# broadinstitute/gatk-bwamem-jni

Measured on AMD Instinct MI355X. Metric: 150bp reads aligned/sec vs GRCh38-scale reference (1/2/4/8 MI355X), higher is better.
Workload: dtype u8/int32/int64; 1 GPU; 10000000 x 150bp single-end synthetic reads per GPU vs synthetic GRCh38-scale genome (3100000000 bp, 24 contigs, 5% diverged repeats), full index in HBM; reads_per_gpu=10000000, read_len=150, genome_bp=3100000000, genome=iid, response_bytes=542940344, parallelism=read-sharded x1, no collectives, hip_hw_queues=4, paired_end=False

## Files before the change

### gatk-bwamem-jni_amd/csrc/bwamem_types.h

```cpp
#pragma once
#include <stdint.h>
#include <stddef.h>
#include <hip/hip_runtime.h>

struct MemOpt {
    int a, b;
    int o_del, e_del;
    int o_ins, e_ins;
    int pen_unpaired;
    int pen_clip5, pen_clip3;
    int w;
    int zdrop;
    uint64_t max_mem_intv;
    int T;
    int flag;
    int min_seed_len;
    int min_chain_weight;
    int max_chain_extend;
    float split_factor;
    int split_width;
    int max_occ;
    int max_chain_gap;
    int n_threads;
    int chunk_size;
// ... 56 lines not shown
    int64_t rb, re;
    int32_t qb, qe;
    int32_t rid;
    int32_t score, truesc, sub, alt_sc, csub, sub_n, w, seedcov, secondary, secondary_all, seedlen0;
    int32_t n_comp, is_alt;
    float frac_rep;
    int32_t pad_;
    uint64_t hash;
};

struct SwJob { int64_t rb; int32_t read, tag, l_ms, is_rev, tlen, xtra, q_off, pad_; };
struct KswR { int score, te, qe, score2, te2, tb, qb; };

struct DevCounters {
    unsigned long long n_ext, n_lf, n_sa, n_dp_cells, n_ref_bases, n_reads;
    unsigned long long dbg[10];
};

enum { ERR_INTV_CAP = 1, ERR_OUT_CAP = 2, ERR_CIGAR_CAP = 4, ERR_LONG_READ = 8, ERR_SCRATCH = 16, ERR_BTREE = 32, ERR_BAD_REG = 64, ERR_JOB_CAP = 128, ERR_ZPOOL = 256, ERR_RESCUE_CAP = 512 };

#define BT_NODE_INTS 40

struct TileView {
    int32_t n_reads;
    int32_t max_len;
    int64_t read_id0;
    const int64_t* seq_off;
    uint8_t* seq;
    int32_t intv_cap;
    Intv* intv;
    int32_t* n_intv;
// ... 36 lines not shown
```

### gatk-bwamem-jni_amd/csrc/k_cigar.hip

```cpp
#include "dev_common.h"
#include "wave_ops.h"
#include "kernels.h"
#include "post_common.h"

#define NEG_SCAN (-2000000000)

struct GClk { unsigned long long* c; long long t; };
DEV void gclk(GClk& K, int k) { if (K.c) { const long long t = clock64(); if (threadIdx.x == 0) atomicAdd(K.c + k, (unsigned long long)(t - K.t)); K.t = clock64(); } }

struct GLds { int32_t* eh_h; int32_t* eh_e; int32_t* tmpM; int rm; };


static __device__ __forceinline__ int traceback(const uint8_t* z, bool z_lds, int n_col, int w, int tlen, int qlen, int lane, uint32_t* cigar, int cig_cap, int& err, uint8_t* tile, GClk& K)
{
    gclk(K, 5);
    int n = 0;
    int which = 0, i = tlen - 1, k = (i + w + 1 < qlen ? i + w + 1 : qlen) - 1;
    int cur_op = -1;
    uint32_t cur_len = 0;
    bool ovf = false;
#define TB_PUSH(OP, LEN) do { if ((OP) == cur_op) cur_len += (uint32_t)(LEN); else { \
        if (cur_len) { if (n >= cig_cap) ovf = true; else { if (lane == 0) cigar[n] = cur_len << 4 | (uint32_t)cur_op; ++n; } } cur_op = (OP); cur_len = (uint32_t)(LEN); } } while (0)
#define TB_WALK(AVAIL, GET) \
    while (i >= 0 && k >= 0 && !ovf && AVAIL(i, k)) { \
// ... 256 lines not shown
    return score;
}

struct GRowTab { uint32_t p[5]; int n[5]; };
DEV GRowTab g_row_tab(const MemOpt& opt)
{
    GRowTab T;
#pragma unroll
    for (int t = 0; t < 5; ++t) {
        T.p[t] = (uint32_t)(uint8_t)opt.mat[t * 5] | (uint32_t)(uint8_t)opt.mat[t * 5 + 1] << 8 | (uint32_t)(uint8_t)opt.mat[t * 5 + 2] << 16 | (uint32_t)(uint8_t)opt.mat[t * 5 + 3] << 24;
        T.n[t] = opt.mat[t * 5 + 4];
    }
    return T;
}

template <int WMAX>
__global__ void __launch_bounds__(64, 2) k_gcigar_lane(DevIndex ix, MemOpt opt, TileView tv, const DpJob* jobs, DpOut* outs, int n_jobs, uint32_t* cig_pool, int cig_cap,
                                                    uint8_t* zpool, unsigned long long zpool_cap, unsigned long long* zpool_cur)
{
    constexpr int NS = 2 * WMAX + 1;
    constexpr int ZW = (NS + 7) / 8;
    const int job = blockIdx.x * 64 + threadIdx.x;
    if (job >= n_jobs) return;
    const DpJob jb = jobs[job];
    const AlnReg ar = tv.regs[tv.seed_off[jb.read] + jb.reg];
    const uint8_t* query = tv.seq + tv.seq_off[jb.read];
    SeqAcc A; A.q = query + ar.qb; A.qlen = ar.qe - ar.qb; A.rev = ar.rb >= ix.l_pac; A.t0 = ar.rb; A.tlen = (int)(ar.re - ar.rb);
    const int qlen = A.qlen, tlen = A.tlen;
    DpOut o; o.score = 0; o.n_cigar = -1;
    const bool usable = !(qlen <= 0 || ar.rb >= ar.re || (ar.rb < ix.l_pac && ar.re > ix.l_pac) || ar.re > ix.l_pac << 1 || ar.rb < 0);
    int w2 = first_w2(opt, ar), w = 0;
    if (usable) {
        w2 = w2 < opt.w << 2 ? w2 : opt.w << 2;
        int max_ins = div_plus(((qlen + 1) >> 1) * opt.mat[0] - opt.o_ins, opt.e_ins, 1);
        int max_del = div_plus(((qlen + 1) >> 1) * opt.mat[0] - opt.o_del, opt.e_del, 1);
        int max_gap = max_ins > max_del ? max_ins : max_del;
        max_gap = max_gap > 1 ? max_gap : 1;
        int d = tlen - qlen; d = d < 0 ? -d : d;
        w = (max_gap + d + 1) >> 1;
        w = w < w2 ? w : w2;
        const int min_w = d + 3;
        w = w > min_w ? w : min_w;
    }
    const int l_end = qlen - 1 - (tlen - 1 - w);
    uint32_t* z = 0;
    bool take = usable && w <= WMAX && l_end >= 0 && l_end <= 2 * w;
    if (take) {
        const unsigned long long need = ((unsigned long long)tlen * ZW * 4 + 63ull) & ~63ull;
        const unsigned long long at = atomicAdd(zpool_cur, need);
        if (at + need > zpool_cap) { atomicOr(tv.err, ERR_ZPOOL); take = false; }
        else z = (uint32_t*)(zpool + at);
    }
    if (!take) { outs[job] = o; return; }

    const int o_del = opt.o_del, e_del = opt.e_del, o_ins = opt.o_ins, e_ins = opt.e_ins;
    const int oe_del = o_del + e_del, oe_ins = o_ins + e_ins;
    const GRowTab RT = g_row_tab(opt);
    SeqCache sc; seq_cache_init(sc);
    int H[NS], E[NS], Q[NS];
#pragma unroll
    for (int l = 0; l < NS; ++l) {
        const int j0 = l - w;
        H[l] = j0 == 0 ? 0 : (j0 > 0 && j0 <= w ? -(o_ins + e_ins * j0) : MINUS_INF);
        E[l] = MINUS_INF;
        Q[l] = j0 >= 0 && j0 < qlen ? acc_q_c(A, sc, j0) : 4;
    }
    for (int i = 0; i < tlen; ++i) {
        const int tb = acc_t_c(ix, A, sc, i);
        const uint32_t R = tb == 0 ? RT.p[0] : tb == 1 ? RT.p[1] : tb == 2 ? RT.p[2] : tb == 3 ? RT.p[3] : RT.p[4];
        const int Rn = tb == 0 ? RT.n[0] : tb == 1 ? RT.n[1] : tb == 2 ? RT.n[2] : tb == 3 ? RT.n[3] : RT.n[4];
        const int c0 = i - w;
        const int hb = -(o_del + e_del * (i + 1));
        int f = MINUS_INF;
        uint32_t zw[ZW];
#pragma unroll
        for (int k = 0; k < ZW; ++k) zw[k] = 0;
#pragma unroll
        for (int l = 0; l < NS; ++l) {
            const int j = c0 + l;
            const bool act = j >= 0 && j < qlen && l <= 2 * w;
            const int q = Q[l];
            const int s = q < 4 ? (int)(int8_t)(R >> (q << 3)) : Rn;
            const int m = H[l] + s, e = E[l];
            int d = m >= e ? 0 : 1;
            int h = m >= e ? m : e;
            d = h >= f ? d : 2;
            h = h >= f ? h : f;
            const int t = m - oe_del;
            int e2 = e - e_del;
            d |= e2 > t ? 4 : 0;
            e2 = e2 > t ? e2 : t;
            const int t2 = m - oe_ins;
            int f2 = f - e_ins;
            d |= f2 > t2 ? 8 : 0;
            f2 = f2 > t2 ? f2 : t2;
            H[l] = act ? h : (j == -1 ? hb : MINUS_INF);
            if (l > 0) E[l - 1] = act ? e2 : MINUS_INF;
            f = act ? f2 : f;
            zw[l >> 3] |= act ? (uint32_t)d << ((l & 7) << 2) : 0u;
        }
        E[NS - 1] = MINUS_INF;
#pragma unroll
        for (int k = 0; k < ZW; ++k) z[i * ZW + k] = zw[k];
        const int inj = i + 1 - w + NS - 1;
        const int qin = inj >= 0 && inj < qlen ? acc_q_c(A, sc, inj) : 4;
#pragma unroll
        for (int l = 0; l + 1 < NS; ++l) Q[l] = Q[l + 1];
        Q[NS - 1] = qin;
    }
    int score = MINUS_INF;
#pragma unroll
    for (int l = 0; l < NS; ++l) score = l == l_end ? H[l] : score;

    if (!(w2 == opt.w << 2) && score < ar.truesc - opt.a) { outs[job] = o; return; }

    uint32_t* cigar = cig_pool + (size_t)job * cig_cap;
    int n = 0, cur_op = -1, which = 0, i = tlen - 1, k = (i + w + 1 < qlen ? i + w + 1 : qlen) - 1;
    uint32_t cur_len = 0;
    bool ovf = false;
#define TB_PUSH(OP, LEN) do { if ((OP) == cur_op) cur_len += (uint32_t)(LEN); else { \
        if (cur_len) { if (n >= cig_cap) ovf = true; else cigar[n++] = cur_len << 4 | (uint32_t)cur_op; } cur_op = (OP); cur_len = (uint32_t)(LEN); } } while (0)
    while (i >= 0 && k >= 0 && !ovf) {
        const int l = k - (i - w);
        const uint32_t nib = z[i * ZW + (l >> 3)] >> ((l & 7) << 2) & 15u;
        which = which == 0 ? (int)(nib & 3u) : which == 1 ? (int)(nib >> 2 & 1u) : (int)(nib >> 3 & 1u) << 1;
        if (which == 0) { TB_PUSH(0, 1); --i; --k; }
        else if (which == 1) { TB_PUSH(2, 1); --i; }
        else { TB_PUSH(1, 1); --k; }
    }
    if (!ovf && i >= 0) TB_PUSH(2, i + 1);
    if (!ovf && k >= 0) TB_PUSH(1, k + 1);
    if (!ovf) TB_PUSH(-1, 0);
#undef TB_PUSH
    for (int a = 0; a < n >> 1; ++a) { uint32_t tmp = cigar[a]; cigar[a] = cigar[n - 1 - a]; cigar[n - 1 - a] = tmp; }
    if (ovf) { atomicOr(tv.err, ERR_CIGAR_CAP); n = 0; }
    o.score = score; o.n_cigar = n;
    outs[job] = o;
}

template <bool HBM, int MAXCH>
__global__ void __launch_bounds__(64, MAXCH >= 13 ? 2 : 4) k_gcigar(DevIndex ix, MemOpt opt, TileView tv, const DpJob* jobs, DpOut* outs, int n_jobs, uint32_t* cig_pool, int cig_cap,
                                               uint8_t* zpool, unsigned long long zpool_cap, unsigned long long* zpool_cur, int z_lds_cap, int ring,
                                               uint8_t* slabs, unsigned long long slab_bytes, int* queue)
{
    HIP_DYNAMIC_SHARED(int32_t, smem)
    const int lane = threadIdx.x;
  for (int job = blockIdx.x, first = 1; ; first = 0) {
    if (slabs) { int nx = 0; if (lane == 0) nx = atomicAdd(queue, 1); job = __shfl(nx, 0); }
    else if (!first) job += HBM ? (int)gridDim.x : n_jobs;
    if (job >= n_jobs) break;
    __syncthreads();
    if (outs[job].n_cigar >= 0) continue;
// ... 66 lines not shown
            else if (MAXCH >= 4 && diag_ok && nch <= 4) score = global_wave_diag_n<4>(ix, opt, sq, lane, A, w, z, z == z_lds, n_col);
            else if (MAXCH >= 7 && diag_ok && nch <= 7) score = global_wave_diag_n<7>(ix, opt, sq, lane, A, w, z, z == z_lds, n_col);
            else if (MAXCH >= 13 && diag_ok && nch <= 13) score = global_wave_diag_n<13>(ix, opt, sq, lane, A, w, z, z == z_lds, n_col);
            else score = global_wave(ix, opt, L, lane, A, w, z, z == z_lds, n_col);
            n_cigar = traceback(z, z == z_lds, n_col, w, rlen, l_query, lane, cigar, cig_cap, err, tile, K);
            __syncthreads();
            if (score == last_sc || w2 == opt.w << 2) break;
            last_sc = score;
            w2 <<= 1;
        } while (++i < 3 && score < ar.truesc - opt.a);
    }
    if (lane == 0 && !deferred) {
        DpOut o; o.score = score; o.n_cigar = n_cigar;
        outs[job] = o;
        if (err) atomicOr(tv.err, err);
    }
  }
}

size_t gcigar_slab_bytes(const MemOpt& opt, int max_len)
{
    if (max_len <= 1000) return 0;
    const size_t w_max = 4 * (size_t)(opt.w > 0 ? opt.w : 0) + 3;
    return ((2 * w_max + 1) * ((size_t)max_len + 2 * w_max + 64) + 255) & ~(size_t)255;
}
int gcigar_slab_grid(const DevIndex& ix, int n_jobs) { const int g = (ix.n_cu > 0 ? ix.n_cu : 256) * 8; return n_jobs < g ? n_jobs : g; }

void launch_gcigar(hipStream_t st, const DevIndex& ix, const MemOpt& opt, const TileView& tv, int n_jobs, const void* jobs, void* outs, uint32_t* cig_pool, int cig_cap,
                   uint8_t* zpool, unsigned long long zpool_cap, unsigned long long* zpool_cur, uint8_t* slabs, size_t slab_bytes, int* queue)
{
    if (n_jobs <= 0) return;
    int z_lds_cap = 6144;
    { const char* e = getenv("BWAMEM_HIP_ZLDS"); if (e && atoi(e) >= 0) z_lds_cap = atoi(e); }
    size_t cap = (size_t)tv.max_len + 2;
    int ring = 64;
    {
        long long need = 8ll * (opt.w > 0 ? opt.w : 0) + 16;
        if (need > (long long)cap) need = (long long)cap;
        if (need > 4096) need = 4096;
        { const char* e = getenv("BWAMEM_HIP_GCIGAR_RING"); if (e && atoi(e) > 0 && atoi(e) < need) need = atoi(e); }
        if (slab_bytes) need = 64;
        while (ring < need) ring <<= 1;
    }
    const size_t tail = ((cap + 15) & ~(size_t)15) + (size_t)z_lds_cap + 64;
    hipLaunchKernelGGL(k_gcigar_lane<16>, dim3((n_jobs + 63) / 64), dim3(64), 0, st, ix, opt, tv, (const DpJob*)jobs, (DpOut*)outs, n_jobs, cig_pool, cig_cap, zpool, zpool_cap, zpool_cur);
    if (!tv.gcigar_hbm_only) {
        if (!slab_bytes) slabs = nullptr;
        const int grid = slabs ? gcigar_slab_grid(ix, n_jobs) : n_jobs;
        if (slabs) hipLaunchKernelGGL((k_gcigar<false, 13>), dim3(grid), dim3(64), 3 * (size_t)ring * sizeof(int32_t) + tail, st, ix, opt, tv, (const DpJob*)jobs, (DpOut*)outs, n_jobs, cig_pool, cig_cap, zpool, zpool_cap, zpool_cur, z_lds_cap, ring,
                                      slabs, (unsigned long long)slab_bytes, queue);
        else hipLaunchKernelGGL((k_gcigar<false, 2>), dim3(grid), dim3(64), 3 * (size_t)ring * sizeof(int32_t) + tail, st, ix, opt, tv, (const DpJob*)jobs, (DpOut*)outs, n_jobs, cig_pool, cig_cap, zpool, zpool_cap, zpool_cur, z_lds_cap, ring,
                                (uint8_t*)nullptr, 0ull, queue);
    }
    if (tv.dp_rows) {
        const int grid = n_jobs < tv.dp_rows_blocks ? n_jobs : tv.dp_rows_blocks;
        hipLaunchKernelGGL((k_gcigar<true, 13>), dim3(grid), dim3(64), tail, st, ix, opt, tv, (const DpJob*)jobs, (DpOut*)outs, n_jobs, cig_pool, cig_cap, zpool, zpool_cap, zpool_cur, z_lds_cap, 0, (uint8_t*)nullptr, 0ull, (int*)nullptr);
    }
}
```

### gatk-bwamem-jni_amd/csrc/kernels.h

```cpp
#pragma once
#include <hip/hip_runtime.h>
#include "bwamem_types.h"
#include "bam_encode.h"

void launch_build_occ64(hipStream_t st, const uint32_t* bwt, uint64_t n_blocks, uint4* occ);
void launch_sa_densify(hipStream_t st, const DevIndex& ix, const uint64_t* sa_src, uint64_t n_src, int src_intv, uint32_t* lo, uint8_t* hi, int32_t* err);
void launch_encode(hipStream_t st, uint8_t* seq, int64_t n_bytes);
void launch_unpack_pac(hipStream_t st, const DevIndex& ix, int64_t start, int64_t n, uint8_t* dst);
void launch_seed(hipStream_t st, const DevIndex& ix, const MemOpt& opt, const TileView& tv);
size_t scan_tmp_bytes(int64_t n);
void launch_scan(hipStream_t st, const int32_t* in, int64_t* out, int n, int64_t* tmp);
void launch_order(hipStream_t st, const int32_t* n_seeds, int n, int32_t* bins64, int32_t* order);
size_t nul_tmp_bytes(int64_t n_bytes);
void launch_nul_offsets(hipStream_t st, const uint8_t* seq, int64_t n_bytes, int64_t* off, int64_t n_reads_max, int64_t* n_found, void* tmp);
void launch_sa(hipStream_t st, const DevIndex& ix, const MemOpt& opt, const TileView& tv, int64_t n_occ);
void launch_chain(hipStream_t st, const DevIndex& ix, const MemOpt& opt, const TileView& tv, Chain* chain_store);
bool rescore_needed(const MemOpt& opt, const TileView& tv);
void launch_rescore(hipStream_t st, const DevIndex& ix, const MemOpt& opt, const TileView& tv, void* jobs, void* results, int32_t* first_num, int32_t* cnt, int cap);
size_t extend_lds_bytes(const MemOpt& opt, int max_len);
void launch_extend(hipStream_t st, const DevIndex& ix, const MemOpt& opt, const TileView& tv);
void launch_post1(hipStream_t st, const DevIndex& ix, const MemOpt& opt, const TileView& tv);
void launch_final_prep(hipStream_t st, const DevIndex& ix, const MemOpt& opt, const TileView& tv);
size_t gcigar_slab_bytes(const MemOpt& opt, int max_len);
int gcigar_slab_grid(const DevIndex& ix, int n_jobs);
void launch_gcigar(hipStream_t st, const DevIndex& ix, const MemOpt& opt, const TileView& tv, int n_jobs, const void* jobs, void* outs, uint32_t* cig_pool, int cig_cap,
                   uint8_t* zpool, unsigned long long zpool_cap, unsigned long long* zpool_cur, uint8_t* slabs, size_t slab_bytes, int* queue);
void launch_final_se(hipStream_t st, const DevIndex& ix, const MemOpt& opt, const TileView& tv, const void* job_out, const uint32_t* job_cig, int cig_cap);
void launch_pack(hipStream_t st, const TileView& tv, uint8_t* dst);
void launch_bam_size(hipStream_t st, const BamTile& t);
void launch_bam_emit(hipStream_t st, const BamTile& t);
int bgzf_grid(int n_cu, int64_t n_blocks);
size_t bgzf_token_bytes(int grid);
void launch_bgzf_deflate(hipStream_t st, const uint8_t* src, int64_t n, int n_blocks, int grid, uint8_t* slots, int32_t* sizes, uint32_t* tokens);
void launch_bgzf_gather(hipStream_t st, const uint8_t* slots, const int32_t* sizes, const int64_t* off, int n_blocks, bool with_eof, uint8_t* out);

void launch_pestat_cand(hipStream_t st, const DevIndex& ix, const MemOpt& opt, const TileView& tv, int8_t* cand_dir, int64_t* cand_is);
void launch_pe_caps(hipStream_t st, const MemOpt& opt, const TileView& tv, int32_t* caps);
void launch_pe_copy_regs(hipStream_t st, const TileView& tv, const AlnReg* src, const int64_t* src_off, AlnReg* dst, const int64_t* dst_off, const int32_t* n_regs);
void launch_pe_pair(hipStream_t st, const DevIndex& ix, const MemOpt& opt, const TileView& tv, AlnReg* regs, const int64_t* reg_off,
                    int32_t* n_regs, int32_t* ints, void* vpool, void* keys, uint8_t* scratch, int64_t scratch_per_pair, int cap_h, int cap_b, int cap_u, const MemPestat* pes, const PairTab& ptab, void* states,
                    void* rescue_jobs, void* rescue_res, int32_t* rescue_first, int32_t* rescue_num, int32_t* rescue_cnt, int rescue_cap);
// ... 6 lines not shown
```

### gatk-bwamem-jni_amd/csrc/pipeline.cpp

```cpp
#include <hip/hip_runtime.h>
#include <stdio.h>
#include <stdlib.h>
#include <string.h>
#include <math.h>
#include <unistd.h>
#include <fcntl.h>
#include <errno.h>
#include <time.h>
#include <sys/stat.h>
#include <sys/mman.h>
#include <dlfcn.h>
#include <mutex>
#include <condition_variable>
#include <thread>
#include <atomic>
#include <functional>
#include <memory>
#include <string>
#include <vector>
#include <deque>
#include <stdexcept>
#include <algorithm>
#include <cmath>
#include "bwamem_types.h"
// ... 55 lines not shown
    const bool forced = e && !strcmp(e, "hbm");
    ext_hbm = forced || extend_lds_bytes(opt, L) + 64 > (size_t)lds;
    gcigar_hbm_only = forced || (size_t)L + 4 + 3 * 1024 * 4 + 6144 + 64 > (size_t)lds;
    need_rows = forced || ext_hbm || gcigar_hbm_only || (long long)L + 4 > 8ll * (opt.w > 0 ? opt.w : 0) + 16 || getenv("BWAMEM_HIP_GCIGAR_RING") != nullptr;
}

struct Workspace {
    int T = 0, L = 0, intv_cap = 0, smem_cap = 0, out_cap = 0;
    int64_t seed_cap = 0, post_per_read = 0;
    DevBuf intv, n_intv, smem, l_rep, n_seeds, seed_off, intv_seed_off;
    DevBuf seeds, seed_rid, cseeds, chains, chain_store, n_chains, bt_nodes, srt, regs, n_regs;
    DevBuf out, out_len, out_off, post, err, cnt;
    DevBuf dp_rows; int dp_rows_blocks = 0;
    bool ext_hbm = false, gcigar_hbm_only = false;
    DevBuf jobs, job_out, job_cig, job_cnt, zpool, zslabs;
    size_t zslab_bytes = 0;
    int job_cap = 0, job_cig_cap = 0; size_t zpool_cap = 0;
    int out_cap_hint = 512;
    int dev_lds = 0;
    DevBuf scan_tmp, packed, order;
    DevBuf pe_dir, pe_is, pe_caps, pe_reg_off2, pe_regs2, pe_ints2, pe_vpool, pe_scratch, pe_states, pe_rescue[3];
    hipStream_t stream = nullptr;
    std::vector<Timed> timed;
    ~Workspace() { if (stream) (void)hipStreamDestroy(stream); }

    bool ensure_reads(const MemOpt& opt, int T_, int L_, int intv_cap_, int out_cap_, int64_t post_per_read_, bool with_seed = true) {
        T = T_; L = L_; intv_cap = intv_cap_; smem_cap = L_ + 2; out_cap = out_cap_; post_per_read = post_per_read_;
        size_t t = (size_t)T;
        if (with_seed && !(intv.ensure(t * intv_cap * sizeof(Intv)) && n_intv.ensure(t * 4) && smem.ensure(((t + 63) / 64 * 64) * 2 * smem_cap * 16)
            && l_rep.ensure(t * 4) && n_seeds.ensure(t * 4) && intv_seed_off.ensure(t * intv_cap * 4))) return false;
        dp_rows_blocks = 0; ext_hbm = gcigar_hbm_only = false;
        bool need_rows = false;
        if (!with_seed) dp_rows_policy(dev_lds, opt, L, need_rows, ext_hbm, gcigar_hbm_only);
        if (need_rows) {
            const size_t per_block = 3 * ((size_t)L + 2) * 4;
            dp_rows_blocks = (int)std::min<size_t>(4096, std::max<size_t>(256, ((size_t)2 << 30) / per_block));
            if (!dp_rows.ensure((size_t)dp_rows_blocks * per_block)) return false;
        }
        return seed_off.ensure((t + 1) * 8) && scan_tmp.ensure(scan_tmp_bytes((int64_t)t + 1)) && order.ensure(t * 4 + 64 * 4)
            && n_chains.ensure(t * 4) && n_regs.ensure(t * 4) && out.ensure(t * out_cap) && out_len.ensure(t * 4)
            && out_off.ensure((t + 1) * 8) && post.ensure(t * (size_t)post_per_read) && err.ensure(64) && cnt.ensure(sizeof(DevCounters));
    }
    bool ensure_jobs(int n_jobs, int cig_cap_, size_t zpool_bytes) {
        job_cap = std::max(job_cap, n_jobs); job_cig_cap = cig_cap_; zpool_cap = std::max(zpool_cap, zpool_bytes);
        return jobs.ensure((size_t)job_cap * 8) && job_out.ensure((size_t)job_cap * 8) && job_cig.ensure((size_t)job_cap * job_cig_cap * 4)
            && job_cnt.ensure(64) && zpool.ensure(zpool_cap);
    }
    bool ensure_seeds(int64_t n) {
        seed_cap = n;
        size_t s = (size_t)n + 16;
        return seeds.ensure(s * sizeof(Seed)) && seed_rid.ensure(s * 4) && cseeds.ensure(s * sizeof(Seed)) && chains.ensure(s * sizeof(Chain))
            && chain_store.ensure(s * sizeof(Chain)) && bt_nodes.ensure((s / 4 + 3 * (size_t)T + 16) * BT_NODE_INTS * 4) && srt.ensure(s * 8)
            && regs.ensure(s * sizeof(AlnReg));
    }
    TileView view(int T_, int L_, int64_t read_id0, uint8_t* seq, const int64_t* seq_off) const {
        TileView tv; memset(&tv, 0, sizeof tv);
        tv.n_reads = T_; tv.max_len = L_; tv.read_id0 = read_id0; tv.seq = seq; tv.seq_off = seq_off;
        tv.intv_cap = intv_cap; tv.intv = intv.as<Intv>(); tv.n_intv = n_intv.as<int32_t>();
        tv.smem_scratch = smem.as<Intv>(); tv.smem_cap = smem_cap; tv.l_rep = l_rep.as<int32_t>();
        tv.n_seeds = n_seeds.as<int32_t>(); tv.seed_off = seed_off.as<int64_t>(); tv.intv_seed_off = intv_seed_off.as<int32_t>();
        tv.seeds = seeds.as<Seed>(); tv.seed_rid = seed_rid.as<int32_t>(); tv.cseeds = cseeds.as<Seed>();
// ... 598 lines not shown
        if (n_occ + 16 > 0x7fffffff) { fprintf(stderr, "[bwamem_hip] tile with more than 2^31 seed occurrences\n"); return false; }
        int rc = (int)(n_occ + 16);
        if (!rescore_full) {
            static const int cap0 = []{ const char* e = getenv("BWAMEM_HIP_RESCORE_CAP0"); return e && atoi(e) > 0 ? atoi(e) : 0; }();
            if (cap0) rc = cap0;
        }
        if (!(ws.pe_rescue[0].ensure(pe_rescue_bytes(0, rc)) && ws.pe_rescue[1].ensure(pe_rescue_bytes(1, rc)) && ws.pe_rescue[2].ensure((size_t)T * 8 + 64))) return false;
        TIMED(ws, K_CHAIN, launch_rescore(ws.stream, ix->d, opt, tv, ws.pe_rescue[0].p, ws.pe_rescue[1].p, ws.pe_rescue[2].as<int32_t>() + 16, ws.pe_rescue[2].as<int32_t>(), rc));
    }
    TIMED(ws, K_EXTEND, launch_extend(ws.stream, ix->d, opt, tv));
    if (getenv("BWAMEM_HIP_DUMP") && T <= 64) debug_dump(ws, tv, T);
    TIMED(ws, K_POST, launch_post1(ws.stream, ix->d, opt, tv));
    return true;
}

static bool run_gcigar(bwaidx_s* ix, Workspace& ws, const MemOpt& opt, const TileView& tv, int n_jobs)
{
    ws.zslab_bytes = gcigar_slab_bytes(opt, tv.max_len);
    if (ws.zslab_bytes && !ws.zslabs.ensure(ws.zslab_bytes * (size_t)gcigar_slab_grid(ix->d, 1 << 30))) return false;
    TIMED(ws, K_FINAL, launch_gcigar(ws.stream, ix->d, opt, tv, n_jobs, ws.jobs.p, ws.job_out.p, ws.job_cig.as<uint32_t>(), ws.job_cig_cap,
                                     ws.zpool.as<uint8_t>(), (unsigned long long)ws.zpool_cap, (unsigned long long*)(ws.job_cnt.as<int32_t>() + 2),
                                     ws.zslabs.as<uint8_t>(), ws.zslab_bytes, ws.job_cnt.as<int32_t>() + 4));
    return true;
}

static bool run_tile_se(bwaidx_s* ix, Workspace& ws, const MemOpt& opt, bwamem_batch_s* b, int64_t read_id0, size_t tile_index, const TileSpec& spec,
                        TileOut& to, const SeedStore& seeds_of_chunk, uint32_t chunk_r0, int& out_cap)
{
    RoctxRange rr("bwamem_hip:tile_se");
    const uint32_t r0 = spec.r0;
    const int T = (int)(spec.r1 - spec.r0), L = spec.L;
    int attempts = 0, job_cap_hint = 0;
    bool rescore_full = false;
    size_t zpool_hint = (size_t)64 << 20;
    double zmult = 1;
    { int oc = 0; ix->hints.get(T, job_cap_hint, zmult, oc); out_cap = std::max(out_cap, oc); }
    for (;;) {
// ... 24 lines not shown
        HIP_OK(hipMemcpyAsync(&n_jobs, tv.job_cnt, 4, hipMemcpyDeviceToHost, ws.stream));
        HIP_OK(hipStreamSynchronize(ws.stream));
        if (n_jobs > ws.job_cap) { job_cap_hint = n_jobs + n_jobs / 4; { std::lock_guard<std::mutex> lk(g_stats.mu); ++g_stats.s.n_retries; } continue; }
        if (!run_gcigar(ix, ws, opt, tv, n_jobs)) return false;
        TIMED(ws, K_FINAL, launch_final_se(ws.stream, ix->d, opt, tv, ws.job_out.p, ws.job_cig.as<uint32_t>(), ws.job_cig_cap));
        TIMED(ws, K_OTHER, launch_scan(ws.stream, tv.out_len, tv.out_off, T, ws.scan_tmp.as<int64_t>()));
        int64_t out_total = 0;
        DevCounters hc;
        int32_t errv[8] = {0, 0, 0, 0, 0, 0, 0, 0};
        HIP_OK(hipMemcpyAsync(&out_total, tv.out_off + T, 8, hipMemcpyDeviceToHost, ws.stream));
        HIP_OK(hipMemcpyAsync(&hc, tv.cnt, sizeof hc, hipMemcpyDeviceToHost, ws.stream));
        HIP_OK(hipMemcpyAsync(errv, tv.err, sizeof errv, hipMemcpyDeviceToHost, ws.stream));
        HIP_OK(hipStreamSynchronize(ws.stream));
        const int32_t err = errv[0];
        if (tv.debug & 0x2000) fprintf(stderr, "[bwamem_hip] global alignment, Mclk summed over waves: rows %.1f tile staging %.1f walk %.1f end %.1f | jobs %d\n", hc.dbg[5] / 1e6, hc.dbg[6] / 1e6, hc.dbg[7] / 1e6, hc.dbg[8] / 1e6, n_jobs);
        if (err) {
            { std::lock_guard<std::mutex> lk(g_stats.mu); ++g_stats.s.n_retries; }
            if (err & ERR_RESCUE_CAP) { if (rescore_full) { fprintf(stderr, "[bwamem_hip] internal error: seed re-scoring list beyond the seed count\n"); return false; } rescore_full = true; continue; }
            if (err & ERR_BAD_REG) { fprintf(stderr, "[bwamem_hip] internal error: extension produced an invalid region (tile read %d of call read %lld: n=%d qb=%d qe=%d rb=%d re=%d score=%d)\n", errv[1], (long long)(read_id0 + r0 + errv[1]), errv[2], errv[3], errv[4], errv[5], errv[6], errv[7]); return false; }
            if (err & ERR_LONG_READ) { fprintf(stderr, "[bwamem_hip] reads long enough to need seed re-scoring (mem_flt_chained_seeds) are not supported on the device path yet\n"); return false; }
            if (err & ERR_BTREE) { fprintf(stderr, "[bwamem_hip] internal error: chain B-tree pool exhausted\n"); return false; }
            if ((err & (ERR_SCRATCH | ERR_CIGAR_CAP)) && !(err & (ERR_ZPOOL | ERR_JOB_CAP))) { fprintf(stderr, "[bwamem_hip] internal error: post-processing scratch exhausted (err=%d)\n", err); return false; }
            if (err & ERR_OUT_CAP) { out_cap *= 4; continue; }
            if (err & ERR_ZPOOL) { zpool_hint = std::max(zpool_hint * 4, ws.zpool_cap * 4); continue; }
            if (err & ERR_JOB_CAP) { job_cap_hint = std::max(ws.job_cap * 2, 4096); continue; }
            fprintf(stderr, "[bwamem_hip] device error flags %d\n", err); return false;
        }
        if (!emit_tile(ws, b, tile_index, tv, out_total, to)) return false;
        ix->hints.learn(T, n_jobs, zpool_hint > ((size_t)64 << 20) ? (double)zpool_hint / ((double)std::max(job_cap_hint, std::max(1024, T / 4)) * (2.0 * L + 64) * 20 + (double)((size_t)64 << 20)) : 1.0, out_cap);
        {
// ... 313 lines not shown
        if ((err & ERR_JOB_CAP) || n_jobs > ws.job_cap) { pe_job_cap = std::max(n_jobs + n_jobs / 4, ws.job_cap * 2); continue; }
        if (err & ERR_SCRATCH) { cap_u *= 8; if (attempts < 4) continue; }
        if (err) { fprintf(stderr, "[bwamem_hip] device error flags %d in the paired-end pairing stage\n", err); return false; }
        {
            TileView tvj = tv;
            tvj.regs = regs2; tvj.seed_off = reg_off2;
            if (!run_gcigar(ix, ws, opt, tvj, n_jobs)) return false;
        }
        TIMED(ws, K_FINAL, launch_pe_out(ws.stream, ix->d, opt, tv, regs2, reg_off2, tv.n_regs, ws.pe_ints2.as<int32_t>(), pes, ws.pe_states.p,
                                         ws.job_out.p, ws.job_cig.as<uint32_t>(), ws.job_cig_cap));
        TIMED(ws, K_OTHER, launch_scan(ws.stream, tv.out_len, tv.out_off, T, ws.scan_tmp.as<int64_t>()));
        int64_t out_total = 0;
        HIP_OK(hipMemcpyAsync(&out_total, tv.out_off + T, 8, hipMemcpyDeviceToHost, ws.stream));
        HIP_OK(hipMemcpyAsync(&err, tv.err, 4, hipMemcpyDeviceToHost, ws.stream));
        HIP_OK(hipStreamSynchronize(ws.stream));
        if (err & ERR_OUT_CAP) { ws.out_cap_hint *= 4; continue; }
        if (err & ERR_ZPOOL) { pe_zpool = std::max(pe_zpool * 4, ws.zpool_cap * 4); continue; }
        if (err) { fprintf(stderr, "[bwamem_hip] device error flags %d in the paired-end phase 2\n", err); return false; }
        if (!emit_tile(ws, b, tile_index, tv, out_total, to)) return false;
        timed_collect(ws);
        return true;
    }
}

static bool pe_begin(bwaidx_s* ix, const MemOpt& opt, const MemPestat* pes0, bwamem_batch_s* b, int64_t read_id0)
{
    b->pe.reset();
    if (pes0 && !build_pair_tab(ix, pes0)) return false;
    PeCall* pc = new PeCall();
    b->pe.reset(pc);
// ... 715 lines not shown
```

### include/bwamem_hip.h

```cpp
#ifndef BWAMEM_HIP_H_
#define BWAMEM_HIP_H_

#include <stddef.h>
#include <stdint.h>

#ifdef __cplusplus
extern "C" {
#endif

typedef struct bwaidx_s bwaidx_t;
typedef struct mem_opt_s mem_opt_t;
typedef struct mem_pestat_s mem_pestat_t;

int jnibwa_createReferenceIndex(const char* refFileName, const char* indexPrefix, const char* algoName);

int jnibwa_createIndexFile(const char* refName, const char* imgName);

bwaidx_t* jnibwa_openIndex(int fd);

int jnibwa_destroyIndex(bwaidx_t* pIdx);

void* jnibwa_getRefContigNames(bwaidx_t* pIdx, size_t* pBufSize);

void* jnibwa_createAlignments(bwaidx_t* pIdx, mem_opt_t* pOpts, mem_pestat_t* peStats, char* pSeq, size_t* pBufSize);
// ... 45 lines not shown
int    bwamem_hip_batch_bgzf_download(bwamem_batch_t* b, void* dst);
void*  bwamem_hip_bgzf_compress_device(bwaidx_t* idx, const void* src, size_t n, int with_eof, size_t* pBytes);
int    bwamem_hip_align_to_bam_device(bwaidx_t* idx, const mem_opt_t* opt, const mem_pestat_t* pes, const char* pSeq, size_t nBytes,
                                      const char* const* readNames, int fd, int write_header);

typedef struct {
    uint64_t n_reads, n_ext, n_lf, n_sa, n_dp_cells;
    double ms_encode, ms_seed, ms_sa, ms_chain, ms_extend, ms_post, ms_final, ms_pack, ms_other;
    uint64_t n_launch_seed, n_launch_sa, n_launch_extend;
    uint64_t n_tiles, n_retries;
} bwamem_stats_t;

void bwamem_hip_stats_enable(int on);
void bwamem_hip_stats_reset(void);
void bwamem_hip_stats_get(bwamem_stats_t* out);

#ifdef __cplusplus
}
#endif
#endif
```

Measured before the change: 23.18 million reads/s.

## Add band-widening retries and a second wider-band lane pass for global CIGAR jobs

Moves the per-lane global alignment into a helper that can retry with a doubled band inside the lane kernel. Jobs that still miss, or whose band exceeds 16, are compacted with a wave ballot into a list. A second lane kernel with WMAX=32 then processes that list, so fewer jobs fall through to the slower wave-per-job slab kernel. Query codes are packed into bytes for wide bands to limit register use, and debug class counters are added. The cost is an extra launch, more register pressure at WMAX=32, and repeated DP rounds for some jobs.

```diff
diff --git a/gatk-bwamem-jni_amd/csrc/bwamem_types.h b/gatk-bwamem-jni_amd/csrc/bwamem_types.h
--- a/gatk-bwamem-jni_amd/csrc/bwamem_types.h
+++ b/gatk-bwamem-jni_amd/csrc/bwamem_types.h
@@ -94,7 +94,7 @@
 
 struct DevCounters {
     unsigned long long n_ext, n_lf, n_sa, n_dp_cells, n_ref_bases, n_reads;
-    unsigned long long dbg[10];
+    unsigned long long dbg[24];
 };
 
 enum { ERR_INTV_CAP = 1, ERR_OUT_CAP = 2, ERR_CIGAR_CAP = 4, ERR_LONG_READ = 8, ERR_SCRATCH = 16, ERR_BTREE = 32, ERR_BAD_REG = 64, ERR_JOB_CAP = 128, ERR_ZPOOL = 256, ERR_RESCUE_CAP = 512 };
diff --git a/gatk-bwamem-jni_amd/csrc/k_cigar.hip b/gatk-bwamem-jni_amd/csrc/k_cigar.hip
--- a/gatk-bwamem-jni_amd/csrc/k_cigar.hip
+++ b/gatk-bwamem-jni_amd/csrc/k_cigar.hip
@@ -294,107 +294,141 @@
     return T;
 }
 
+DEV int gen_cigar_band(const MemOpt& opt, int qlen, int tlen, int w2)
+{
+    int max_ins = div_plus(((qlen + 1) >> 1) * opt.mat[0] - opt.o_ins, opt.e_ins, 1);
+    int max_del = div_plus(((qlen + 1) >> 1) * opt.mat[0] - opt.o_del, opt.e_del, 1);
+    int max_gap = max_ins > max_del ? max_ins : max_del;
+    max_gap = max_gap > 1 ? max_gap : 1;
+    int d = tlen - qlen; d = d < 0 ? -d : d;
+    int w = (max_gap + d + 1) >> 1;
+    w = w < w2 ? w : w2;
+    const int min_w = d + 3;
+    return w > min_w ? w : min_w;
+}
+
+struct GLanePool { uint8_t* base; unsigned long long cap; unsigned long long* cur; };
+
+enum { GL_KEPT = 0, GL_KEPT_RETRIED = 1, GL_HANDED_ON = 2, GL_WIDE = 3, GL_UNUSABLE = 4, GL_NO_POOL = 5 };
+
+template <int NS, bool PACKED> struct GLaneQ;
+template <int NS> struct GLaneQ<NS, false> {
+    int q[NS];
+    __device__ __forceinline__ void set(int l, int code) { q[l] = code << 3; }
+    __device__ __forceinline__ int get(int l) const { return q[l]; }
+    __device__ __forceinline__ void slide(int code) {
+#pragma unroll
+        for (int l = 0; l + 1 < NS; ++l) q[l] = q[l + 1];
+        q[NS - 1] = code << 3;
+    }
+};
+template <int NS> struct GLaneQ<NS, true> {
+    static constexpr int QW = (NS + 3) / 4;
+    uint32_t q[QW];
+    __device__ __forceinline__ void set(int l, int code) { const int k = l >> 2, s = (l & 3) << 3; q[k] = (q[k] & ~(0xffu << s)) | (uint32_t)(code << 3) << s; }
+    __device__ __forceinline__ int get(int l) const { return (int)(q[l >> 2] >> ((l & 3) << 3) & 0xffu); }
+    __device__ __forceinline__ void slide(int code) {
+#pragma unroll
+        for (int k = 0; k + 1 < QW; ++k) q[k] = q[k] >> 8 | q[k + 1] << 24;
+        q[QW - 1] = (q[QW - 1] >> 8 & ~(0xffu << (((NS - 1) & 3) << 3))) | (uint32_t)(code << 3) << (((NS - 1) & 3) << 3);
+    }
+};
+
 template <int WMAX>
-__global__ void __launch_bounds__(64, 2) k_gcigar_lane(DevIndex ix, MemOpt opt, TileView tv, const DpJob* jobs, DpOut* outs, int n_jobs, uint32_t* cig_pool, int cig_cap,
-                                                    uint8_t* zpool, unsigned long long zpool_cap, unsigned long long* zpool_cur)
+DEV int gcigar_lane_job(const DevIndex& ix, const MemOpt& opt, const SeqAcc& A, bool usable, int w2, int truesc, bool retries, const GLanePool& zp,
+                        uint32_t* cigar, int cig_cap, DpOut& o, int& err)
 {
     constexpr int NS = 2 * WMAX + 1;
     constexpr int ZW = (NS + 7) / 8;
-    const int job = blockIdx.x * 64 + threadIdx.x;
-    if (job >= n_jobs) return;
-    const DpJob jb = jobs[job];
-    const AlnReg ar = tv.regs[tv.seed_off[jb.read] + jb.reg];
-    const uint8_t* query = tv.seq + tv.seq_off[jb.read];
-    SeqAcc A; A.q = query + ar.qb; A.qlen = ar.qe - ar.qb; A.rev = ar.rb >= ix.l_pac; A.t0 = ar.rb; A.tlen = (int)(ar.re - ar.rb);
     const int qlen = A.qlen, tlen = A.tlen;
-    DpOut o; o.score = 0; o.n_cigar = -1;
-    const bool usable = !(qlen <= 0 || ar.rb >= ar.re || (ar.rb < ix.l_pac && ar.re > ix.l_pac) || ar.re > ix.l_pac << 1 || ar.rb < 0);
-    int w2 = first_w2(opt, ar), w = 0;
-    if (usable) {
-        w2 = w2 < opt.w << 2 ? w2 : opt.w << 2;
-        int max_ins = div_plus(((qlen + 1) >> 1) * opt.mat[0] - opt.o_ins, opt.e_ins, 1);
-        int max_del = div_plus(((qlen + 1) >> 1) * opt.mat[0] - opt.o_del, opt.e_del, 1);
-        int max_gap = max_ins > max_del ? max_ins : max_del;
-        max_gap = max_gap > 1 ? max_gap : 1;
-        int d = tlen - qlen; d = d < 0 ? -d : d;
-        w = (max_gap + d + 1) >> 1;
-        w = w < w2 ? w : w2;
-        const int min_w = d + 3;
-        w = w > min_w ? w : min_w;
-    }
-    const int l_end = qlen - 1 - (tlen - 1 - w);
-    uint32_t* z = 0;
-    bool take = usable && w <= WMAX && l_end >= 0 && l_end <= 2 * w;
-    if (take) {
+    o.score = 0; o.n_cigar = -1;
+    int w = 0;
+    if (usable) { w2 = w2 < opt.w << 2 ? w2 : opt.w << 2; w = gen_cigar_band(opt, qlen, tlen, w2); }
+    int l_end = qlen - 1 - (tlen - 1 - w);
+    if (!usable || l_end < 0 || l_end > 2 * w) return GL_UNUSABLE;
+    if (w > WMAX) return GL_WIDE;
+    uint32_t* z;
+    {
         const unsigned long long need = ((unsigned long long)tlen * ZW * 4 + 63ull) & ~63ull;
-        const unsigned long long at = atomicAdd(zpool_cur, need);
-        if (at + need > zpool_cap) { atomicOr(tv.err, ERR_ZPOOL); take = false; }
-        else z = (uint32_t*)(zpool + at);
-    }
-    if (!take) { outs[job] = o; return; }
+        const unsigned long long at = atomicAdd(zp.cur, need);
+        if (at + need > zp.cap) { err |= ERR_ZPOOL; return GL_NO_POOL; }
+        z = (uint32_t*)(zp.base + at);
+    }
 
     const int o_del = opt.o_del, e_del = opt.e_del, o_ins = opt.o_ins, e_ins = opt.e_ins;
     const int oe_del = o_del + e_del, oe_ins = o_ins + e_ins;
     const GRowTab RT = g_row_tab(opt);
     SeqCache sc; seq_cache_init(sc);
-    int H[NS], E[NS], Q[NS];
-#pragma unroll
-    for (int l = 0; l < NS; ++l) {
-        const int j0 = l - w;
-        H[l] = j0 == 0 ? 0 : (j0 > 0 && j0 <= w ? -(o_ins + e_ins * j0) : MINUS_INF);
-        E[l] = MINUS_INF;
-        Q[l] = j0 >= 0 && j0 < qlen ? acc_q_c(A, sc, j0) : 4;
-    }
-    for (int i = 0; i < tlen; ++i) {
-        const int tb = acc_t_c(ix, A, sc, i);
-        const uint32_t R = tb == 0 ? RT.p[0] : tb == 1 ? RT.p[1] : tb == 2 ? RT.p[2] : tb == 3 ? RT.p[3] : RT.p[4];
-        const int Rn = tb == 0 ? RT.n[0] : tb == 1 ? RT.n[1] : tb == 2 ? RT.n[2] : tb == 3 ? RT.n[3] : RT.n[4];
-        const int c0 = i - w;
-        const int hb = -(o_del + e_del * (i + 1));
-        int f = MINUS_INF;
-        uint32_t zw[ZW];
-#pragma unroll
-        for (int k = 0; k < ZW; ++k) zw[k] = 0;
+    int score = MINUS_INF, last_sc = -(1 << 30), round = 0;
+    for (;;) {
+        int H[NS], E[NS];
+        GLaneQ<NS, (NS > 33)> Q;
+        if (NS > 33) {
+#pragma unroll
+            for (int k = 0; k < (NS + 3) / 4; ++k) Q.q[k] = 0;
+        }
 #pragma unroll
         for (int l = 0; l < NS; ++l) {
-            const int j = c0 + l;
-            const bool act = j >= 0 && j < qlen && l <= 2 * w;
-            const int q = Q[l];
-            const int s = q < 4 ? (int)(int8_t)(R >> (q << 3)) : Rn;
-            const int m = H[l] + s, e = E[l];
-            int d = m >= e ? 0 : 1;
-            int h = m >= e ? m : e;
-            d = h >= f ? d : 2;
-            h = h >= f ? h : f;
-            const int t = m - oe_del;
-            int e2 = e - e_del;
-            d |= e2 > t ? 4 : 0;
-            e2 = e2 > t ? e2 : t;
-            const int t2 = m - oe_ins;
-            int f2 = f - e_ins;
-            d |= f2 > t2 ? 8 : 0;
-            f2 = f2 > t2 ? f2 : t2;
-            H[l] = act ? h : (j == -1 ? hb : MINUS_INF);
-            if (l > 0) E[l - 1] = act ? e2 : MINUS_INF;
-            f = act ? f2 : f;
-            zw[l >> 3] |= act ? (uint32_t)d << ((l & 7) << 2) : 0u;
-        }
-        E[NS - 1] = MINUS_INF;
-#pragma unroll
-        for (int k = 0; k < ZW; ++k) z[i * ZW + k] = zw[k];
-        const int inj = i + 1 - w + NS - 1;
-        const int qin = inj >= 0 && inj < qlen ? acc_q_c(A, sc, inj) : 4;
-#pragma unroll
-        for (int l = 0; l + 1 < NS; ++l) Q[l] = Q[l + 1];
-        Q[NS - 1] = qin;
-    }
-    int score = MINUS_INF;
-#pragma unroll
-    for (int l = 0; l < NS; ++l) score = l == l_end ? H[l] : score;
-
-    if (!(w2 == opt.w << 2) && score < ar.truesc - opt.a) { outs[job] = o; return; }
-
-    uint32_t* cigar = cig_pool + (size_t)job * cig_cap;
+            const int j0 = l - w;
+            H[l] = j0 == 0 ? 0 : (j0 > 0 && j0 <= w ? -(o_ins + e_ins * j0) : MINUS_INF);
+            E[l] = MINUS_INF;
+            Q.set(l, j0 >= 0 && j0 < qlen ? acc_q_c(A, sc, j0) : 4);
+        }
+        for (int i = 0; i < tlen; ++i) {
+            const int tb = acc_t_c(ix, A, sc, i);
+            const uint32_t R = tb == 0 ? RT.p[0] : tb == 1 ? RT.p[1] : tb == 2 ? RT.p[2] : tb == 3 ? RT.p[3] : RT.p[4];
+            const int Rn = tb == 0 ? RT.n[0] : tb == 1 ? RT.n[1] : tb == 2 ? RT.n[2] : tb == 3 ? RT.n[3] : RT.n[4];
+            const int c0 = i - w;
+            const int hb = -(o_del + e_del * (i + 1));
+            const int lo = c0 < 0 ? -c0 : 0, hi = qlen - c0 < 2 * w + 1 ? qlen - c0 : 2 * w + 1;
+            const unsigned span = hi > lo ? (unsigned)(hi - lo) : 0u;
+            int f = MINUS_INF;
+            uint32_t zw[ZW];
+#pragma unroll
+            for (int k = 0; k < ZW; ++k) zw[k] = 0;
+#pragma unroll
+            for (int l = 0; l < NS; ++l) {
+                const int j = c0 + l;
+                const bool act = (unsigned)(l - lo) < span;
+                const int q8 = Q.get(l);
+                const int s = q8 < 32 ? (int)(int8_t)(R >> q8) : Rn;
+                const int m = H[l] + s, e = E[l];
+                int d = m >= e ? 0 : 1;
+                int h = m >= e ? m : e;
+                d = h >= f ? d : 2;
+                h = h >= f ? h : f;
+                const int t = m - oe_del;
+                int e2 = e - e_del;
+                d |= e2 > t ? 4 : 0;
+                e2 = e2 > t ? e2 : t;
+                const int t2 = m - oe_ins;
+                int f2 = f - e_ins;
+                d |= f2 > t2 ? 8 : 0;
+                f2 = f2 > t2 ? f2 : t2;
+                H[l] = act ? h : (j == -1 ? hb : MINUS_INF);
+                if (l > 0) E[l - 1] = act ? e2 : MINUS_INF;
+                f = act ? f2 : f;
+                zw[l >> 3] |= act ? (uint32_t)d << ((l & 7) << 2) : 0u;
+            }
+            E[NS - 1] = MINUS_INF;
+#pragma unroll
+            for (int k = 0; k < ZW; ++k) z[i * ZW + k] = zw[k];
+            const int inj = i + 1 - w + NS - 1;
+            Q.slide(inj >= 0 && inj < qlen ? acc_q_c(A, sc, inj) : 4);
+        }
+        score = MINUS_INF;
+#pragma unroll
+        for (int l = 0; l < NS; ++l) score = l == l_end ? H[l] : score;
+
+        if (score == last_sc || w2 == opt.w << 2 || round + 1 >= 3 || !(score < truesc - opt.a)) break;
+        if (!retries) return GL_HANDED_ON;
+        last_sc = score; w2 <<= 1; ++round;
+        w2 = w2 < opt.w << 2 ? w2 : opt.w << 2;
+        w = gen_cigar_band(opt, qlen, tlen, w2);
+        l_end = qlen - 1 - (tlen - 1 - w);
+        if (w > WMAX || l_end < 0 || l_end > 2 * w) return GL_HANDED_ON;
+    }
+
     int n = 0, cur_op = -1, which = 0, i = tlen - 1, k = (i + w + 1 < qlen ? i + w + 1 : qlen) - 1;
     uint32_t cur_len = 0;
     bool ovf = false;
@@ -413,9 +447,55 @@
     if (!ovf) TB_PUSH(-1, 0);
 #undef TB_PUSH
     for (int a = 0; a < n >> 1; ++a) { uint32_t tmp = cigar[a]; cigar[a] = cigar[n - 1 - a]; cigar[n - 1 - a] = tmp; }
-    if (ovf) { atomicOr(tv.err, ERR_CIGAR_CAP); n = 0; }
+    if (ovf) { err |= ERR_CIGAR_CAP; n = 0; }
     o.score = score; o.n_cigar = n;
+    return round ? GL_KEPT_RETRIED : GL_KEPT;
+}
+
+template <int WMAX>
+DEV bool gcigar_lane_run(const DevIndex& ix, const MemOpt& opt, const TileView& tv, const DpJob* jobs, DpOut* outs, int job, bool retries, uint32_t* cig_pool, int cig_cap,
+                         const GLanePool& zp)
+{
+    const DpJob jb = jobs[job];
+    const AlnReg ar = tv.regs[tv.seed_off[jb.read] + jb.reg];
+    const uint8_t* query = tv.seq + tv.seq_off[jb.read];
+    SeqAcc A; A.q = query + ar.qb; A.qlen = ar.qe - ar.qb; A.rev = ar.rb >= ix.l_pac; A.t0 = ar.rb; A.tlen = (int)(ar.re - ar.rb);
+    const bool usable = !(A.qlen <= 0 || ar.rb >= ar.re || (ar.rb < ix.l_pac && ar.re > ix.l_pac) || ar.re > ix.l_pac << 1 || ar.rb < 0);
+    DpOut o;
+    int err = 0;
+    const int cls = gcigar_lane_job<WMAX>(ix, opt, A, usable, first_w2(opt, ar), ar.truesc, retries, zp, cig_pool + (size_t)job * cig_cap, cig_cap, o, err);
     outs[job] = o;
+    if (err) atomicOr(tv.err, err);
+    if (tv.debug & 0x2000) atomicAdd(&tv.cnt->dbg[(WMAX > 16 ? 16 : 10) + cls], 1ull);
+    return o.n_cigar >= 0;
+}
+
+template <int WMAX>
+__global__ void __launch_bounds__(64, 2) k_gcigar_lane(DevIndex ix, MemOpt opt, TileView tv, const DpJob* jobs, DpOut* outs, int n_jobs, uint32_t* cig_pool, int cig_cap,
+                                                    uint8_t* zpool, unsigned long long zpool_cap, unsigned long long* zpool_cur, int* left, int* left_cnt)
+{
+    const int job = blockIdx.x * 64 + threadIdx.x;
+    GLanePool zp; zp.base = zpool; zp.cap = zpool_cap; zp.cur = zpool_cur;
+    const bool open = job < n_jobs && !gcigar_lane_run<WMAX>(ix, opt, tv, jobs, outs, job, left != nullptr, cig_pool, cig_cap, zp);
+    if (!left) return;
+    const unsigned long long om = __ballot(open);
+    if (om) {
+        const int l_ = threadIdx.x & 63, src = __ffsll((long long)om) - 1;
+        int base = 0;
+        if (l_ == src) base = atomicAdd(left_cnt, __popcll(om));
+        base = __shfl(base, src);
+        if (open) left[base + __popcll(om & ((1ull << l_) - 1ull))] = job;
+    }
+}
+
+template <int WMAX>
+__global__ void __launch_bounds__(64, 2) k_gcigar_lane_list(DevIndex ix, MemOpt opt, TileView tv, const DpJob* jobs, DpOut* outs, uint32_t* cig_pool, int cig_cap,
+                                                         uint8_t* zpool, unsigned long long zpool_cap, unsigned long long* zpool_cur, const int* left, const int* left_cnt)
+{
+    const int n_left = *left_cnt;
+    GLanePool zp; zp.base = zpool; zp.cap = zpool_cap; zp.cur = zpool_cur;
+    for (int idx = blockIdx.x * 64 + threadIdx.x; idx < n_left; idx += gridDim.x * 64)
+        gcigar_lane_run<WMAX>(ix, opt, tv, jobs, outs, left[idx], true, cig_pool, cig_cap, zp);
 }
 
 template <bool HBM, int MAXCH>
@@ -512,6 +592,7 @@
         DpOut o; o.score = score; o.n_cigar = n_cigar;
         outs[job] = o;
         if (err) atomicOr(tv.err, err);
+        if (K.c) atomicAdd(K.c + 22, 1ull);
     }
   }
 }
@@ -525,7 +606,7 @@
 int gcigar_slab_grid(const DevIndex& ix, int n_jobs) { const int g = (ix.n_cu > 0 ? ix.n_cu : 256) * 8; return n_jobs < g ? n_jobs : g; }
 
 void launch_gcigar(hipStream_t st, const DevIndex& ix, const MemOpt& opt, const TileView& tv, int n_jobs, const void* jobs, void* outs, uint32_t* cig_pool, int cig_cap,
-                   uint8_t* zpool, unsigned long long zpool_cap, unsigned long long* zpool_cur, uint8_t* slabs, size_t slab_bytes, int* queue)
+                   uint8_t* zpool, unsigned long long zpool_cap, unsigned long long* zpool_cur, uint8_t* slabs, size_t slab_bytes, int* queue, int* left, int* left_cnt)
 {
     if (n_jobs <= 0) return;
     int z_lds_cap = 6144;
@@ -541,7 +622,12 @@
         while (ring < need) ring <<= 1;
     }
     const size_t tail = ((cap + 15) & ~(size_t)15) + (size_t)z_lds_cap + 64;
-    hipLaunchKernelGGL(k_gcigar_lane<16>, dim3((n_jobs + 63) / 64), dim3(64), 0, st, ix, opt, tv, (const DpJob*)jobs, (DpOut*)outs, n_jobs, cig_pool, cig_cap, zpool, zpool_cap, zpool_cur);
+    if (slab_bytes) left = nullptr;
+    hipLaunchKernelGGL(k_gcigar_lane<16>, dim3((n_jobs + 63) / 64), dim3(64), 0, st, ix, opt, tv, (const DpJob*)jobs, (DpOut*)outs, n_jobs, cig_pool, cig_cap, zpool, zpool_cap, zpool_cur, left, left_cnt);
+    if (left) {
+        const int full = (ix.n_cu > 0 ? ix.n_cu : 256) * 8, need = (n_jobs + 63) / 64;
+        hipLaunchKernelGGL(k_gcigar_lane_list<32>, dim3(need < full ? need : full), dim3(64), 0, st, ix, opt, tv, (const DpJob*)jobs, (DpOut*)outs, cig_pool, cig_cap, zpool, zpool_cap, zpool_cur, left, left_cnt);
+    }
     if (!tv.gcigar_hbm_only) {
         if (!slab_bytes) slabs = nullptr;
         const int grid = slabs ? gcigar_slab_grid(ix, n_jobs) : n_jobs;
diff --git a/gatk-bwamem-jni_amd/csrc/kernels.h b/gatk-bwamem-jni_amd/csrc/kernels.h
--- a/gatk-bwamem-jni_amd/csrc/kernels.h
+++ b/gatk-bwamem-jni_amd/csrc/kernels.h
@@ -24,7 +24,7 @@
 size_t gcigar_slab_bytes(const MemOpt& opt, int max_len);
 int gcigar_slab_grid(const DevIndex& ix, int n_jobs);
 void launch_gcigar(hipStream_t st, const DevIndex& ix, const MemOpt& opt, const TileView& tv, int n_jobs, const void* jobs, void* outs, uint32_t* cig_pool, int cig_cap,
-                   uint8_t* zpool, unsigned long long zpool_cap, unsigned long long* zpool_cur, uint8_t* slabs, size_t slab_bytes, int* queue);
+                   uint8_t* zpool, unsigned long long zpool_cap, unsigned long long* zpool_cur, uint8_t* slabs, size_t slab_bytes, int* queue, int* left, int* left_cnt);
 void launch_final_se(hipStream_t st, const DevIndex& ix, const MemOpt& opt, const TileView& tv, const void* job_out, const uint32_t* job_cig, int cig_cap);
 void launch_pack(hipStream_t st, const TileView& tv, uint8_t* dst);
 void launch_bam_size(hipStream_t st, const BamTile& t);
diff --git a/gatk-bwamem-jni_amd/csrc/pipeline.cpp b/gatk-bwamem-jni_amd/csrc/pipeline.cpp
--- a/gatk-bwamem-jni_amd/csrc/pipeline.cpp
+++ b/gatk-bwamem-jni_amd/csrc/pipeline.cpp
@@ -93,6 +93,7 @@
     DevBuf dp_rows; int dp_rows_blocks = 0;
     bool ext_hbm = false, gcigar_hbm_only = false;
     DevBuf jobs, job_out, job_cig, job_cnt, zpool, zslabs;
+    DevBuf job_left;
     size_t zslab_bytes = 0;
     int job_cap = 0, job_cig_cap = 0; size_t zpool_cap = 0;
     int out_cap_hint = 512;
@@ -123,7 +124,7 @@
     bool ensure_jobs(int n_jobs, int cig_cap_, size_t zpool_bytes) {
         job_cap = std::max(job_cap, n_jobs); job_cig_cap = cig_cap_; zpool_cap = std::max(zpool_cap, zpool_bytes);
         return jobs.ensure((size_t)job_cap * 8) && job_out.ensure((size_t)job_cap * 8) && job_cig.ensure((size_t)job_cap * job_cig_cap * 4)
-            && job_cnt.ensure(64) && zpool.ensure(zpool_cap);
+            && job_cnt.ensure(64) && zpool.ensure(zpool_cap) && job_left.ensure((size_t)job_cap * 4);
     }
     bool ensure_seeds(int64_t n) {
         seed_cap = n;
@@ -752,13 +753,29 @@
     return true;
 }
 
+static std::mutex g_gclass_mu;
+static unsigned long long g_gclass[13];
+static void gcigar_classes_add(const DevCounters& hc, int n_jobs)
+{
+    std::lock_guard<std::mutex> lk(g_gclass_mu);
+    for (int k = 0; k < 13; ++k) g_gclass[k] += hc.dbg[10 + k];
+    fprintf(stderr, "[bwamem_hip] global alignment jobs %d | 33 slots: kept %llu, kept after retries %llu, handed on %llu, wider %llu, unusable %llu, no pool %llu"
+                    " | 65 slots: kept %llu, kept after retries %llu, handed on %llu, wider %llu, unusable %llu, no pool %llu | wave form %llu\n", n_jobs,
+            hc.dbg[10], hc.dbg[11], hc.dbg[12], hc.dbg[13], hc.dbg[14], hc.dbg[15], hc.dbg[16], hc.dbg[17], hc.dbg[18], hc.dbg[19], hc.dbg[20], hc.dbg[21], hc.dbg[22]);
+}
+void bwamem_hip_gcigar_classes(unsigned long long* out13, int reset)
+{
+    std::lock_guard<std::mutex> lk(g_gclass_mu);
+    for (int k = 0; k < 13; ++k) { if (out13) out13[k] = g_gclass[k]; if (reset) g_gclass[k] = 0; }
+}
+
 static bool run_gcigar(bwaidx_s* ix, Workspace& ws, const MemOpt& opt, const TileView& tv, int n_jobs)
 {
     ws.zslab_bytes = gcigar_slab_bytes(opt, tv.max_len);
     if (ws.zslab_bytes && !ws.zslabs.ensure(ws.zslab_bytes * (size_t)gcigar_slab_grid(ix->d, 1 << 30))) return false;
     TIMED(ws, K_FINAL, launch_gcigar(ws.stream, ix->d, opt, tv, n_jobs, ws.jobs.p, ws.job_out.p, ws.job_cig.as<uint32_t>(), ws.job_cig_cap,
                                      ws.zpool.as<uint8_t>(), (unsigned long long)ws.zpool_cap, (unsigned long long*)(ws.job_cnt.as<int32_t>() + 2),
-                                     ws.zslabs.as<uint8_t>(), ws.zslab_bytes, ws.job_cnt.as<int32_t>() + 4));
+                                     ws.zslabs.as<uint8_t>(), ws.zslab_bytes, ws.job_cnt.as<int32_t>() + 4, ws.job_left.as<int32_t>(), ws.job_cnt.as<int32_t>() + 6));
     return true;
 }
 
@@ -813,6 +830,7 @@
         HIP_OK(hipStreamSynchronize(ws.stream));
         const int32_t err = errv[0];
         if (tv.debug & 0x2000) fprintf(stderr, "[bwamem_hip] global alignment, Mclk summed over waves: rows %.1f tile staging %.1f walk %.1f end %.1f | jobs %d\n", hc.dbg[5] / 1e6, hc.dbg[6] / 1e6, hc.dbg[7] / 1e6, hc.dbg[8] / 1e6, n_jobs);
+        if (tv.debug & 0x2000) gcigar_classes_add(hc, n_jobs);
         if (err) {
             { std::lock_guard<std::mutex> lk(g_stats.mu); ++g_stats.s.n_retries; }
             if (err & ERR_RESCUE_CAP) { if (rescore_full) { fprintf(stderr, "[bwamem_hip] internal error: seed re-scoring list beyond the seed count\n"); return false; } rescore_full = true; continue; }
@@ -1156,6 +1174,7 @@
         HIP_OK(hipMemcpyAsync(&out_total, tv.out_off + T, 8, hipMemcpyDeviceToHost, ws.stream));
         HIP_OK(hipMemcpyAsync(&err, tv.err, 4, hipMemcpyDeviceToHost, ws.stream));
         HIP_OK(hipStreamSynchronize(ws.stream));
+        if (tv.debug & 0x2000) { DevCounters hc; HIP_OK(hipMemcpy(&hc, tv.cnt, sizeof hc, hipMemcpyDeviceToHost)); gcigar_classes_add(hc, n_jobs); }
         if (err & ERR_OUT_CAP) { ws.out_cap_hint *= 4; continue; }
         if (err & ERR_ZPOOL) { pe_zpool = std::max(pe_zpool * 4, ws.zpool_cap * 4); continue; }
         if (err) { fprintf(stderr, "[bwamem_hip] device error flags %d in the paired-end phase 2\n", err); return false; }
diff --git a/include/bwamem_hip.h b/include/bwamem_hip.h
--- a/include/bwamem_hip.h
+++ b/include/bwamem_hip.h
@@ -83,6 +83,7 @@
 void bwamem_hip_stats_enable(int on);
 void bwamem_hip_stats_reset(void);
 void bwamem_hip_stats_get(bwamem_stats_t* out);
+void bwamem_hip_gcigar_classes(unsigned long long* out13, int reset);
 
 #ifdef __cplusplus
 }
```

After: 22.80 million reads/s. -1.7%, worse.
